# travelingspaceman/LowThrustOpt

Measured on NVIDIA B200. Metric: segment-propagations/s (fp64 state+STM), higher is better.
Workload: dtype f64

## Files before the change

lowthrustopt_b200/csrc/lto_direct_cw.cu:

```cuda
#include "lto_internal.h"
#include "lto_cw_common.cuh"
#include <algorithm>

namespace lto {

namespace cw {

constexpr int NTILE = 2;
constexpr int NSLOT = 2;
constexpr int XW0 = 2;

template <int NS>
struct Cfg {
    static constexpr int NCOL = NS + 3;
    static constexpr int NW = NTILE + NCOL;
    static constexpr int NTHREADS = 32 * NW;
    static constexpr int SVAL = (NS == 7) ? 10 : 6;
    static constexpr int OFF_H = 13 * SVAL;
    static constexpr int OFF_BM = OFF_H + 1;
    static constexpr int STEP_DOUBLES = OFF_BM + ((NS == 7) ? 3 : 0);
    static constexpr size_t REC_BYTES = (size_t)NTILE * NSLOT * STEP_DOUBLES * 32 * sizeof(double);
    static constexpr int NV = 2 * (NS + 3);
    static constexpr size_t OUT_TILE_BYTES = (size_t)16 * NS * NV * sizeof(double);
    static constexpr size_t OUT_BYTES = (size_t)NTILE * OUT_TILE_BYTES;
    static constexpr size_t BAR_OFF = REC_BYTES + OUT_BYTES;
    static constexpr size_t FLAG_OFF = BAR_OFF + (size_t)NTILE * NSLOT * 2 * sizeof(unsigned long long);
    static constexpr size_t PARK_OFF = (FLAG_OFF + (size_t)NTILE * NSLOT * sizeof(int) + 15) & ~(size_t)15;
    static constexpr int NPARK = (NS == 7) ? 7 : 6;
    static constexpr size_t SMEM = PARK_OFF + (size_t)NTILE * NCOL * NPARK * 32 * sizeof(double);
};

enum { K1P_WORK, K1P_BAR, K1P_PACE, K1P_STORE, K1P_TOTAL, K1P_STEPS, K1P_N };
#ifdef LTO_K1_PROF
constexpr int K1P_MAX_BLOCKS = 1024, K1P_MAX_WARPS = 16;
__device__ unsigned long long k1_prof[K1P_MAX_BLOCKS * K1P_MAX_WARPS * K1P_N];
struct K1Prof {
    long long c[K1P_N], t, t_begin;
    __device__ __forceinline__ void start() {
        for (int i = 0; i < K1P_N; ++i) c[i] = 0;
        t = t_begin = clock64();
    }
    __device__ __forceinline__ void mark() { t = clock64(); }
    __device__ __forceinline__ void add(int i) { const long long n = clock64(); c[i] += n - t; t = n; }
    __device__ __forceinline__ void step() { ++c[K1P_STEPS]; }
    __device__ __forceinline__ void flush(int warp, int lane) {
        c[K1P_TOTAL] = clock64() - t_begin;
        if (lane == 0 && blockIdx.x < K1P_MAX_BLOCKS)
            for (int i = 0; i < K1P_N; ++i) k1_prof[((size_t)blockIdx.x * K1P_MAX_WARPS + warp) * K1P_N + i] = (unsigned long long)c[i];
    }
};
#else
struct K1Prof {
    __device__ __forceinline__ void start() {}
    __device__ __forceinline__ void mark() {}
    __device__ __forceinline__ void add(int) {}
    __device__ __forceinline__ void step() {}
    __device__ __forceinline__ void flush(int, int) {}
};
#endif

using namespace cwc;

template <int NS, bool PUB = true>
__device__ __forceinline__ double x_step(double (&r)[3], double (&v)[3], double& m, const double (&u)[3], double omega,
                                         double mdot, double h, const EPConst& c, double* __restrict__ rec, double* __restrict__ stg,
                                         double& maxErr) {
    constexpr int SVAL = Cfg<NS>::SVAL;
    const double h2 = h * h;
    const double w2 = 2.0 * omega;
    const double kom6 = c.kthr / c.default_mass;
    double a[13][3];
    double ev[3] = {0.0, 0.0, 0.0}, ea[3] = {0.0, 0.0, 0.0};
    if (PUB) rec[Cfg<NS>::OFF_H * 32] = h;
#pragma unroll
    for (int j = 0; j < 13; ++j) {
        double R[3], V[3];
#pragma unroll
        for (int q = 0; q < 3; ++q) {
            double accv = 0.0, accr = 0.0;
#pragma unroll
            for (int l = 0; l < j; ++l) {
                if (lto_tab::Bf(j, l) != 0.0) accv = fma(lto_tab::Bf(j, l), a[l][q], accv);
                if (lto_tab::Gf(j, l) != 0.0) accr = fma(lto_tab::Gf(j, l), a[l][q], accr);
            }
            V[q] = (j == 0) ? v[q] : fma(h, accv, v[q]);
            R[q] = (j == 0) ? r[q] : fma(h2, accr, fma(h * lto_tab::Cf(j), v[q], r[q]));
        }
        const double dx1 = R[0] + c.mu, dx2 = dx1 - 1.0;
        const double yz = fma(R[1], R[1], R[2] * R[2]);
        const double i1 = fast_rsqrt(fma(dx1, dx1, yz));
        const double i2 = fast_rsqrt(fma(dx2, dx2, yz));
        const double i1s = i1 * i1, i2s = i2 * i2;
        const double a31 = c.m1 * i1s * i1, a32 = c.mu * i2s * i2;
        const double gg1 = 1.0 - (a31 + a32);
        double kom = kom6, im = 0.0;
        if (NS == 7) { im = fast_rcp(fma(h * lto_tab::Cf(j), mdot, m)); kom = c.kthr * im; }
        a[j][0] = fma(u[0], kom, fma(-a31, dx1, fma(-a32, dx2, fma(w2, V[1], R[0]))));
        a[j][1] = fma(u[1], kom, fma(gg1, R[1], -w2 * V[0]));
        a[j][2] = fma(u[2], kom, (gg1 - 1.0) * R[2]);
        if (PUB && j != 10) {
            const double a51 = 3.0 * i1s * a31, a52 = 3.0 * i2s * a32;
            const double s5 = a51 + a52;
            const double p1 = a51 * dx1, p2 = a52 * dx2;
            const double t = p1 + p2;
            const double s5y = s5 * R[1];
            double2* w = reinterpret_cast<double2*>(stg + j * SVAL * 32);
            w[0] = make_double2(fma(p1, dx1, fma(p2, dx2, gg1)), fma(s5y, R[1], gg1));
            w[1] = make_double2(fma(s5 * R[2], R[2], gg1 - 1.0), t * R[1]);
            w[2] = make_double2(t * R[2], s5y * R[2]);
            if (NS == 7) {
                const double k2 = -kom * im;
                w[3] = make_double2(kom, k2 * u[0]);
                w[4] = make_double2(k2 * u[1], k2 * u[2]);
            }
        }
        if (lto_tab::PSIf(j) != 0.0) {
#pragma unroll
            for (int q = 0; q < 3; ++q) { ev[q] = fma(lto_tab::PSIf(j), V[q], ev[q]); ea[q] = fma(lto_tab::PSIf(j), a[j][q], ea[q]); }
        }
    }
    double delta = 0.0;
#pragma unroll
    for (int q = 0; q < 3; ++q) {
        double sv = 0.0, sr = 0.0;
#pragma unroll
        for (int l = 0; l < 13; ++l) {
            if (lto_tab::CHIf(l) != 0.0) sv = fma(lto_tab::CHIf(l), a[l][q], sv);
            if (lto_tab::CHIBf(l) != 0.0) sr = fma(lto_tab::CHIBf(l), a[l][q], sr);
        }
        r[q] = fma(h2, sr, fma(h, v[q], r[q]));
        v[q] = fma(h, sv, v[q]);
        delta = fmax(delta, fmax(fabs(ev[q]), fabs(ea[q])));
    }
    if (NS == 7) m = fma(h, mdot, m);
    delta *= fabs(h * lto_tab::ERRC);
    maxErr = fmax(maxErr, delta);
    return delta;
}

template <int NS>
__device__ __forceinline__ void col_step(double (&sr)[3], double (&sv)[3], double& sm, double bm, int gc,
                                         double omega, double kom6, const double* __restrict__ rec, const double* __restrict__ stg) {
    constexpr int SVAL = Cfg<NS>::SVAL;
    constexpr bool MASS = (NS == 7);
    const double h = rec[Cfg<NS>::OFF_H * 32];
    const double h2 = h * h;
    const double w2 = 2.0 * omega;
    double a[13][3];
#pragma unroll
    for (int j = 0; j < 13; ++j) {
        if (j == 10) continue;
        double R[3], V[3];
#pragma unroll
        for (int q = 0; q < 3; ++q) {
            double accv = 0.0, accr = 0.0;
#pragma unroll
            for (int l = 0; l < j; ++l) {
                if (lto_tab::Bf(j, l) != 0.0) accv = fma(lto_tab::Bf(j, l), a[l][q], accv);
                if (lto_tab::Gf(j, l) != 0.0) accr = fma(lto_tab::Gf(j, l), a[l][q], accr);
            }
            V[q] = (j == 0) ? sv[q] : fma(h, accv, sv[q]);
            R[q] = (j == 0) ? sr[q] : fma(h2, accr, fma(h * lto_tab::Cf(j), sv[q], sr[q]));
        }
        const double2* w = reinterpret_cast<const double2*>(stg + j * SVAL * 32);
        const double2 w0 = w[0], w1 = w[1], w2v = w[2];
        const double U[6] = {w0.x, w0.y, w1.x, w1.y, w2v.x, w2v.y};
        double2 w3 = make_double2(kom6, 0.0), w4 = make_double2(0.0, 0.0);
        if (MASS) { w3 = w[3]; w4 = w[4]; }
        const double kom = w3.x;
        double acc[3];
        acc[0] = fma(w2, V[1], gc == 0 ? kom : 0.0);
        acc[1] = fma(-w2, V[0], gc == 1 ? kom : 0.0);
        acc[2] = gc == 2 ? kom : 0.0;
        if (MASS) {
            const double smj = fma(h * lto_tab::Cf(j), bm, sm);
            const double am[3] = {w3.y, w4.x, w4.y};
#pragma unroll
            for (int q = 0; q < 3; ++q) acc[q] = fma(am[q], smj, acc[q]);
        }
        sym3_mul_acc(U, R, acc);
#pragma unroll
        for (int q = 0; q < 3; ++q) a[j][q] = acc[q];
    }
#pragma unroll
    for (int q = 0; q < 3; ++q) {
        double dv = 0.0, dr = 0.0;
#pragma unroll
        for (int l = 0; l < 13; ++l) {
            if (lto_tab::CHIf(l) != 0.0) dv = fma(lto_tab::CHIf(l), a[l][q], dv);
            if (lto_tab::CHIBf(l) != 0.0) dr = fma(lto_tab::CHIBf(l), a[l][q], dr);
        }
        sr[q] = fma(h2, dr, fma(h, sv[q], sr[q]));
        sv[q] = fma(h, dv, sv[q]);
    }
    if (MASS) sm = fma(h, bm, sm);
}

struct ColState { double sr[3], sv[3], sm; };

template <int NS>
__device__ __forceinline__ void col_init(ColState& c, int col) {
#pragma unroll
    for (int q = 0; q < 3; ++q) { c.sr[q] = (col == q) ? 1.0 : 0.0; c.sv[q] = (col == q + 3) ? 1.0 : 0.0; }
    c.sm = (NS == 7 && col == 6) ? 1.0 : 0.0;
}

template <int NS>
__device__ __forceinline__ void col_park(double* __restrict__ p, const ColState& c) {
#pragma unroll
    for (int q = 0; q < 3; ++q) { p[q * 32] = c.sr[q]; p[(3 + q) * 32] = c.sv[q]; }
    if (NS == 7) p[6 * 32] = c.sm;
}

template <int NS>
__device__ __forceinline__ void col_unpark(const double* __restrict__ p, ColState& c) {
#pragma unroll
    for (int q = 0; q < 3; ++q) { c.sr[q] = p[q * 32]; c.sv[q] = p[(3 + q) * 32]; }
    c.sm = (NS == 7) ? p[6 * 32] : 0.0;
}

template <int NS>
__device__ __forceinline__ void col_store(double* __restrict__ stage, const ColState& c, int col, int lane) {
    constexpr int NV = 2 * (NS + 3);
    const int back = lane & 1, gc = col - NS;
    const int ocol = (gc >= 0) ? (2 * NS + (back ? 3 : 0) + gc) : ((back ? NS : 0) + col);
    double* J = stage + (lane >> 1) * (NS * NV) + ocol * NS;
    const double rj = (col >= 3 && col < 6) ? -1.0 : 1.0;
    const double sp = back ? -rj : 1.0;
    const double sq = back ? rj : 1.0;
    J[0] = sp * c.sr[0]; J[1] = sp * c.sr[1]; J[2] = sp * c.sr[2];
    J[3] = sq * c.sv[0]; J[4] = sq * c.sv[1]; J[5] = sq * c.sv[2];
    if (NS == 7) J[6] = sp * c.sm;
}

template <int NS>
__device__ __forceinline__ double* col_park_at(double* parks, int t, int col, int lane) {
    return parks + (size_t)(t * Cfg<NS>::NCOL + col) * Cfg<NS>::NPARK * 32 + lane;
}

template <int NS, bool ADAPT>
__device__ __forceinline__ bool col_tile_step(int t, unsigned g, int col, int gc, int lane, double omega, double kom6, double* recs, double* parks,
                                              unsigned bars, volatile int* lastf, K1Prof& pf) {
    typedef Cfg<NS> C;
    const unsigned slot = g & (NSLOT - 1), par = (g / NSLOT) & 1;
    const double* slotp = recs + (size_t)(t * NSLOT + slot) * C::STEP_DOUBLES * 32;
    const double* rec = slotp + lane;
    const unsigned full = bars + (unsigned)((t * NSLOT + slot) * 16), empty = full + 8;
    mbar_wait(full, par);
    pf.add(K1P_BAR);
    double* park = col_park_at<NS>(parks, t, col, lane);
    ColState cs;
    col_unpark<NS>(park, cs);
    const double bm = (NS == 7 && gc >= 0) ? rec[(C::OFF_BM + gc) * 32] : 0.0;
    const bool last = ADAPT && lastf[t * NSLOT + slot] != 0;
    col_step<NS>(cs.sr, cs.sv, cs.sm, bm, gc, omega, kom6, rec, slotp + lane * C::SVAL);
    mbar_arrive(empty);
    col_park<NS>(park, cs);
    pf.add(K1P_WORK);
    pf.step();
    return last;
}

template <int NS>
__device__ __forceinline__ void col_tiles_store(const DirectArgs& a, long long pair, int col, int lane, double* outs, double* parks) {
    typedef Cfg<NS> C;
    const bool leader = (col == 0 && lane == 0);
#pragma unroll 1
    for (int t = 0; t < NTILE; ++t) {
        const long long seg0 = (pair * NTILE + t) * 16;
        double* stage = outs + (size_t)t * (C::OUT_TILE_BYTES / sizeof(double));
        if (leader) bulk_store_wait_read_but<NTILE - 1>();
        asm volatile("bar.sync 2, %0;" ::"n"(32 * C::NCOL) : "memory");
        ColState cs;
        col_unpark<NS>(col_park_at<NS>(parks, t, col, lane), cs);
        col_store<NS>(stage, cs, col, lane);
        fence_proxy_async();
        asm volatile("bar.sync 2, %0;" ::"n"(32 * C::NCOL) : "memory");
        if (leader && seg0 < a.n_seg) {
            const long long nseg = (a.n_seg - seg0 < 16) ? (a.n_seg - seg0) : 16;
            bulk_store(a.jac + seg0 * (long long)(NS * C::NV), smem_u32(stage), (unsigned)(nseg * NS * C::NV * sizeof(double)));
        }
    }
}

template <int NS>
__device__ __forceinline__ void column_warp(const DirectArgs& a, long long n_tiles, int warp, int col, int lane, double* recs, double* outs, double* parks,
                                            unsigned bars) {
    typedef Cfg<NS> C;
    const int nstep = a.cfg.nsteps - 1;
    const double omega = (lane & 1) ? -1.0 : 1.0;
    const double kom6 = a.c.kthr / a.c.default_mass;
    const int gc = col - NS;
    K1Prof pf;
    pf.start();
    unsigned g = 0;
    for (long long pair = blockIdx.x; pair * NTILE < n_tiles; pair += gridDim.x) {
#pragma unroll 1
        for (int t = 0; t < NTILE; ++t) { ColState c; col_init<NS>(c, col); col_park<NS>(col_park_at<NS>(parks, t, col, lane), c); }
        for (int k = 0; k < nstep; ++k, ++g) {
            pf.mark();
#ifndef LTO_K1_NO_PACE
            asm volatile("bar.sync 3, %0;" ::"n"(32 * C::NCOL) : "memory");
#endif
            pf.add(K1P_PACE);
#pragma unroll 1
            for (int t = 0; t < NTILE; ++t) col_tile_step<NS, false>(t, g, col, gc, lane, omega, kom6, recs, parks, bars, nullptr, pf);
        }
        pf.mark();
        col_tiles_store<NS>(a, pair, col, lane, outs, parks);
        pf.add(K1P_STORE);
    }
    if (col == 0 && lane == 0) bulk_store_wait_all();
    pf.flush(warp, lane);
}

template <int NS>
__device__ __forceinline__ void state_warp(const DirectArgs& a, long long n_tiles, int warp, int t, int lane, double* recs, unsigned bars) {
    typedef Cfg<NS> C;
    const int nsteps = a.cfg.nsteps, nstep = nsteps - 1;
    const int back = lane & 1;
    const double omega = back ? -1.0 : 1.0;
    double r[3], v[3], m = a.c.default_mass, u[3], bm[3] = {0.0, 0.0, 0.0}, mdot = 0.0, t0 = 0.0, t1 = 1.0, maxErr = 0.0;
    K1Prof pf;
    pf.start();
    unsigned g = 0;
    for (long long pair = blockIdx.x; pair * NTILE < n_tiles; pair += gridDim.x) {
        const long long seg = (pair * NTILE + t) * 16 + (lane >> 1);
        {
            const long long sc = seg < a.n_seg ? seg : a.n_seg - 1;
            const long long ia = lto_node_a(sc, a.npt);
            const double* X = (back ? a.Xb : a.Xa) + ia * NS;
            const double* U = (back ? a.ub : a.ua) + ia * 3;
            r[0] = X[0]; r[1] = X[1]; r[2] = X[2];
            v[0] = X[3]; v[1] = X[4]; v[2] = X[5];
            if (back) { v[0] = -v[0]; v[1] = -v[1]; v[2] = -v[2]; }
            if (NS == 7) m = X[6];
            u[0] = U[0]; u[1] = U[1]; u[2] = U[2];
            const double ta = a.ta[ia], tb = a.tb[ia];
            t0 = ta; t1 = ta + (tb - ta) / 2.0;
            const double un = sqrt(fma(u[0], u[0], fma(u[1], u[1], u[2] * u[2])));
            mdot = -omega * un * a.c.cmdot;
            if (NS == 7) {
#pragma unroll
                for (int q = 0; q < 3; ++q) {
                    const double uh = (un > 0.0) ? u[q] / un : 1.0;
                    bm[q] = -omega * a.c.cmdot * uh;
                }
            }
            maxErr = 0.0;
        }
        for (int k = 0; k < nstep; ++k, ++g) {
            const unsigned slot = g & (NSLOT - 1), use = g / NSLOT;
            double* slotp = recs + (size_t)(t * NSLOT + slot) * C::STEP_DOUBLES * 32;
            double* rec = slotp + lane;
            const unsigned full = bars + (unsigned)((t * NSLOT + slot) * 16), empty = full + 8;
            pf.mark();
            if (use > 0) mbar_wait(empty, (use - 1) & 1);
            pf.add(K1P_BAR);
            const double h = linrange_at(t0, t1, nsteps, k + 1) - linrange_at(t0, t1, nsteps, k);
            if (NS == 7) {
#pragma unroll
                for (int q = 0; q < 3; ++q) rec[(C::OFF_BM + q) * 32] = bm[q];
            }
            x_step<NS>(r, v, m, u, omega, mdot, h, a.c, rec, slotp + lane * C::SVAL, maxErr);
            mbar_arrive(full);
            pf.add(K1P_WORK);
            pf.step();
        }
        const unsigned fullmask = 0xffffffffu;
        double xe[NS];
        xe[0] = r[0]; xe[1] = r[1]; xe[2] = r[2];
        xe[3] = back ? -v[0] : v[0]; xe[4] = back ? -v[1] : v[1]; xe[5] = back ? -v[2] : v[2];
        if (NS == 7) xe[6] = m;
        bool bad = false;
#pragma unroll
        for (int q = 0; q < NS; ++q) {
            const double other = __shfl_xor_sync(fullmask, xe[q], 1);
            const double d = xe[q] - other;
            bad |= !(d == d);
            if (!back && seg < a.n_seg) a.defect[seg * NS + q] = d;
        }
        const double me_o = __shfl_xor_sync(fullmask, maxErr, 1);
        if (!back && seg < a.n_seg) {
            if (a.errors) a.errors[seg] = fmax(maxErr, me_o);
            if (a.status) a.status[seg] = bad ? LTO_ST_NAN : LTO_OK;
        }
    }
    pf.flush(warp, lane);
}


template <int NS>
__device__ __forceinline__ void zero_step_record(double* rec, double* stg) {
    constexpr int SVAL = Cfg<NS>::SVAL;
#pragma unroll
    for (int j = 0; j < 13; ++j) {
        double2* w = reinterpret_cast<double2*>(stg + j * SVAL * 32);
#pragma unroll
        for (int p = 0; p < SVAL / 2; ++p) w[p] = make_double2(0.0, 0.0);
    }
    rec[Cfg<NS>::OFF_H * 32] = 0.0;
}

template <int NS>
__device__ __forceinline__ void state_warp_adapt(const DirectArgs& a, long long n_tiles, int t, int lane, double* recs, unsigned bars, volatile int* lastf) {
    typedef Cfg<NS> C;
    const int back = lane & 1;
    const double omega = back ? -1.0 : 1.0;
    const unsigned fullmask = 0xffffffffu;
    double r[3], v[3], m = a.c.default_mass, u[3], bm[3] = {0.0, 0.0, 0.0}, mdot = 0.0, dummy = 0.0;
    unsigned g = 0;
    for (long long pair = blockIdx.x; pair * NTILE < n_tiles; pair += gridDim.x) {
        const long long seg = (pair * NTILE + t) * 16 + (lane >> 1);
        const long long sc = seg < a.n_seg ? seg : a.n_seg - 1;
        const long long ia = lto_node_a(sc, a.npt);
        const double* X = (back ? a.Xb : a.Xa) + ia * NS;
        const double* U = (back ? a.ub : a.ua) + ia * 3;
        r[0] = X[0]; r[1] = X[1]; r[2] = X[2];
        v[0] = X[3]; v[1] = X[4]; v[2] = X[5];
        if (back) { v[0] = -v[0]; v[1] = -v[1]; v[2] = -v[2]; }
        if (NS == 7) m = X[6];
        u[0] = U[0]; u[1] = U[1]; u[2] = U[2];
        const double ta = a.ta[ia], tb = a.tb[ia];
        const double t0 = ta, tfinal = ta + (tb - ta) / 2.0;
        const double un = sqrt(fma(u[0], u[0], fma(u[1], u[1], u[2] * u[2])));
        mdot = -omega * un * a.c.cmdot;
        if (NS == 7) {
#pragma unroll
            for (int q = 0; q < 3; ++q) { const double uh = (un > 0.0) ? u[q] / un : 1.0; bm[q] = -omega * a.c.cmdot * uh; }
        }
        const double hmax = (tfinal - t0) / 2.5, hmin = (tfinal - t0) / 1e7;
        double tt = t0, h = (tfinal - t0) / 50.0;
        int status = 0, nt = 0;
        bool done = !((tt < tfinal) && (h >= hmin));
        while (true) {
            const unsigned slot = g & (NSLOT - 1), use = g / NSLOT;
            double* slotp = recs + (size_t)(t * NSLOT + slot) * C::STEP_DOUBLES * 32;
            double* rec = slotp + lane;
            double* stg = slotp + lane * C::SVAL;
            const unsigned full = bars + (unsigned)((t * NSLOT + slot) * 16), empty = full + 8;
            if (use > 0) mbar_wait(empty, (use - 1) & 1);
            if (NS == 7) {
#pragma unroll
                for (int q = 0; q < 3; ++q) rec[(C::OFF_BM + q) * 32] = bm[q];
            }
            bool pending = !done;
            if (done) {
                zero_step_record<NS>(rec, stg);
            }
            while (__any_sync(fullmask, pending)) {
                if (pending) {
                    if (tt + h > tfinal) h = tfinal - tt;
                    if (nt >= a.cfg.max_attempts) { status = LTO_ST_MAXSTEPS; done = true; pending = false; }
                }
                if (pending) {
                    ++nt;
                    double r2[3] = {r[0], r[1], r[2]}, v2[3] = {v[0], v[1], v[2]}, m2 = m;
                    const double xn = fmax(fmax(fmax(fabs(r[0]), fabs(r[1])), fmax(fabs(r[2]), fabs(v[0]))), fmax(fmax(fabs(v[1]), fabs(v[2])), NS == 7 ? fabs(m) : 0.0));
                    double delta = x_step<NS>(r2, v2, m2, u, omega, mdot, h, a.c, rec, stg, dummy);
                    if (!(delta == delta)) { status = LTO_ST_NAN; done = true; pending = false; }
                    else {
                        const double tau = a.cfg.tol * fmax(xn, 1.0);
                        if (delta <= tau) {
                            tt += h;
                            r[0] = r2[0]; r[1] = r2[1]; r[2] = r2[2]; v[0] = v2[0]; v[1] = v2[1]; v[2] = v2[2]; m = m2;
                            pending = false;
                        }
                        if (delta == 0.0) delta = 1e-16;
                        h = fmin(hmax, 0.8 * h * pow(tau / delta, 0.125));
                        if (!((tt < tfinal) && (h >= hmin))) { done = true; if (pending) { status = LTO_ST_HMIN; pending = false; } }
                    }
                }
            }
            if (status != 0) zero_step_record<NS>(rec, stg);
            const bool all_done = __all_sync(fullmask, done);
            if (lane == 0) lastf[t * NSLOT + slot] = all_done ? 1 : 0;
            mbar_arrive(full);
            ++g;
            if (all_done) break;
        }
        if (status == 0 && tt < tfinal) status = LTO_ST_HMIN;
        double xe[NS];
        xe[0] = r[0]; xe[1] = r[1]; xe[2] = r[2];
        xe[3] = back ? -v[0] : v[0]; xe[4] = back ? -v[1] : v[1]; xe[5] = back ? -v[2] : v[2];
        if (NS == 7) xe[6] = m;
        bool bad = false;
#pragma unroll
        for (int q = 0; q < NS; ++q) {
            const double other = __shfl_xor_sync(fullmask, xe[q], 1);
            const double d = xe[q] - other;
            bad |= !(d == d);
            if (!back && seg < a.n_seg) a.defect[seg * NS + q] = d;
        }
        const int st_o = __shfl_xor_sync(fullmask, status, 1);
        if (!back && seg < a.n_seg) {
            if (a.errors) a.errors[seg] = 0.0;
            if (a.status) a.status[seg] = status ? status : (st_o ? st_o : (bad ? LTO_ST_NAN : LTO_OK));
        }
    }
}

template <int NS>
__device__ __forceinline__ void column_warp_adapt(const DirectArgs& a, long long n_tiles, int warp, int col, int lane, double* recs, double* outs,
                                                  double* parks, unsigned bars, volatile int* lastf) {
    const double omega = (lane & 1) ? -1.0 : 1.0;
    const double kom6 = a.c.kthr / a.c.default_mass;
    const int gc = col - NS;
    K1Prof pf;
    pf.start();
    unsigned g[NTILE];
#pragma unroll
    for (int t = 0; t < NTILE; ++t) g[t] = 0;
    for (long long pair = blockIdx.x; pair * NTILE < n_tiles; pair += gridDim.x) {
#pragma unroll 1
        for (int t = 0; t < NTILE; ++t) { ColState c; col_init<NS>(c, col); col_park<NS>(col_park_at<NS>(parks, t, col, lane), c); }
        unsigned alive = (1u << NTILE) - 1u;
        while (alive) {
            pf.mark();
#ifndef LTO_K1_NO_PACE
            asm volatile("bar.sync 3, %0;" ::"n"(32 * Cfg<NS>::NCOL) : "memory");
#endif
            pf.add(K1P_PACE);
#pragma unroll
            for (int t = 0; t < NTILE; ++t) {
                if (!(alive & (1u << t))) continue;
                if (col_tile_step<NS, true>(t, g[t], col, gc, lane, omega, kom6, recs, parks, bars, lastf, pf)) alive &= ~(1u << t);
                ++g[t];
            }
        }
        pf.mark();
        col_tiles_store<NS>(a, pair, col, lane, outs, parks);
        pf.add(K1P_STORE);
    }
    if (col == 0 && lane == 0) bulk_store_wait_all();
    pf.flush(warp, lane);
}

template <int NS, bool ADAPT>
__global__ void __launch_bounds__(Cfg<NS>::NTHREADS, 1) k_direct_cw(DirectArgs a, long long n_tiles) {
    typedef Cfg<NS> C;
    extern __shared__ __align__(16) unsigned char smem_raw[];
    double* recs = reinterpret_cast<double*>(smem_raw);
    double* outs = reinterpret_cast<double*>(smem_raw + C::REC_BYTES);
    double* parks = reinterpret_cast<double*>(smem_raw + C::PARK_OFF);
    const unsigned bars = smem_u32(smem_raw + C::BAR_OFF);
    const int warp = threadIdx.x >> 5, lane = threadIdx.x & 31;
    if (threadIdx.x == 0) {
#pragma unroll
        for (int i = 0; i < NTILE * NSLOT; ++i) {
            mbar_init(bars + i * 16, 32);
            mbar_init(bars + i * 16 + 8, 32 * C::NCOL);
        }
    }
    __syncthreads();
    volatile int* lastf = reinterpret_cast<volatile int*>(smem_raw + C::FLAG_OFF);
    if (warp >= XW0 && warp < XW0 + NTILE) {
        if (ADAPT) state_warp_adapt<NS>(a, n_tiles, warp - XW0, lane, recs, bars, lastf);
        else state_warp<NS>(a, n_tiles, warp, warp - XW0, lane, recs, bars);
    } else {
        const int col = warp < XW0 ? warp : warp - NTILE;
        if (ADAPT) column_warp_adapt<NS>(a, n_tiles, warp, col, lane, recs, outs, parks, bars, lastf);
        else column_warp<NS>(a, n_tiles, warp, col, lane, recs, outs, parks, bars);
    }
}

template <int NS>
__global__ void __launch_bounds__(128) k_direct_state(DirectArgs a) {
    const int nsteps = a.cfg.nsteps, nstep = nsteps - 1;
    const int lane = threadIdx.x & 31, back = lane & 1;
    const double omega = back ? -1.0 : 1.0;
    const long long n_pairs32 = (a.n_seg + 15) / 16;
    const long long warp0 = ((long long)blockIdx.x * blockDim.x + threadIdx.x) >> 5, nwarp = ((long long)gridDim.x * blockDim.x) >> 5;
    for (long long w = warp0; w < n_pairs32; w += nwarp) {
        const long long seg = w * 16 + (lane >> 1);
        const long long sc = seg < a.n_seg ? seg : a.n_seg - 1;
        const long long ia = lto_node_a(sc, a.npt);
        const double* X = (back ? a.Xb : a.Xa) + ia * NS;
        const double* U = (back ? a.ub : a.ua) + ia * 3;
        double r[3] = {X[0], X[1], X[2]}, v[3] = {X[3], X[4], X[5]}, m = a.c.default_mass, u[3] = {U[0], U[1], U[2]}, maxErr = 0.0;
        if (back) { v[0] = -v[0]; v[1] = -v[1]; v[2] = -v[2]; }
        if (NS == 7) m = X[6];
        const double ta = a.ta[ia], tb = a.tb[ia];
        const double t0 = ta, t1 = ta + (tb - ta) / 2.0;
        const double un = sqrt(fma(u[0], u[0], fma(u[1], u[1], u[2] * u[2])));
        const double mdot = -omega * un * a.c.cmdot;
        for (int k = 0; k < nstep; ++k) {
            const double h = linrange_at(t0, t1, nsteps, k + 1) - linrange_at(t0, t1, nsteps, k);
            x_step<NS, false>(r, v, m, u, omega, mdot, h, a.c, nullptr, nullptr, maxErr);
        }
        const unsigned fullmask = 0xffffffffu;
        double xe[NS];
        xe[0] = r[0]; xe[1] = r[1]; xe[2] = r[2];
        xe[3] = back ? -v[0] : v[0]; xe[4] = back ? -v[1] : v[1]; xe[5] = back ? -v[2] : v[2];
        if (NS == 7) xe[6] = m;
        bool bad = false;
#pragma unroll
        for (int q = 0; q < NS; ++q) {
            const double other = __shfl_xor_sync(fullmask, xe[q], 1);
            const double d = xe[q] - other;
            bad |= !(d == d);
            if (!back && seg < a.n_seg) a.defect[seg * NS + q] = d;
        }
        const double me_o = __shfl_xor_sync(fullmask, maxErr, 1);
        if (!back && seg < a.n_seg) {
            if (a.errors) a.errors[seg] = fmax(maxErr, me_o);
            if (a.status) a.status[seg] = bad ? LTO_ST_NAN : LTO_OK;
        }
    }
}

}

template <int NS>
static cudaError_t launch_state(const DirectArgs& a, cudaStream_t st) {
    int dev = 0, n_sm = 0;
    cudaError_t e = cudaGetDevice(&dev); if (e != cudaSuccess) return e;
    e = cudaDeviceGetAttribute(&n_sm, cudaDevAttrMultiProcessorCount, dev); if (e != cudaSuccess) return e;
    const long long n_warps = (a.n_seg + 15) / 16;
    const long long blocks = (n_warps + 3) / 4;
    const int grid = (int)std::min<long long>(blocks, (long long)n_sm * 16);
    cw::k_direct_state<NS><<<grid, 128, 0, st>>>(a);
    return cudaGetLastError();
}

template <int NS, bool ADAPT>
static cudaError_t launch_cw(const DirectArgs& a, cudaStream_t st) {
    typedef cw::Cfg<NS> C;
    static int n_sm_dev[64] = {0};
    static bool attr_dev[64] = {false};
    int dev = 0;
    { cudaError_t e = cudaGetDevice(&dev); if (e != cudaSuccess) return e; }
    if (dev < 0 || dev >= 64) return cudaErrorInvalidDevice;
    if (!attr_dev[dev]) {
        cudaError_t e = cudaDeviceGetAttribute(&n_sm_dev[dev], cudaDevAttrMultiProcessorCount, dev); if (e != cudaSuccess) return e;
        e = cudaFuncSetAttribute(cw::k_direct_cw<NS, ADAPT>, cudaFuncAttributeMaxDynamicSharedMemorySize, (int)C::SMEM);
        if (e != cudaSuccess) return e;
        attr_dev[dev] = true;
    }
    const int n_sm = n_sm_dev[dev];
    const long long n_tiles = (a.n_seg + 15) / 16;
    const long long n_pairs = (n_tiles + cw::NTILE - 1) / cw::NTILE;
    const int grid = (int)std::min<long long>(n_pairs, (long long)n_sm);
    cw::k_direct_cw<NS, ADAPT><<<grid, C::NTHREADS, C::SMEM, st>>>(a, n_tiles);
    return cudaGetLastError();
}

#ifdef LTO_K1_PROF
extern "C" int lto_k1_prof_read(unsigned long long* out, int n_words) {
    const size_t n = std::min<size_t>((size_t)n_words, sizeof(cw::k1_prof) / sizeof(unsigned long long));
    return (int)cudaMemcpyFromSymbol(out, cw::k1_prof, n * sizeof(unsigned long long));
}
#endif

cudaError_t launch_direct_cw(const DirectArgs& a, int nstate, cudaStream_t st, int* n_launch) {
    *n_launch = 0;
    if (a.n_seg <= 0 || a.n_seg > (1ll << 34)) return cudaErrorNotSupported;
    if (a.cfg.mode != 0 && (a.cfg.err_norm != 0 || a.jac == nullptr)) return cudaErrorNotSupported;
    if (a.jac != nullptr && (reinterpret_cast<uintptr_t>(a.jac) & 15u) != 0) return cudaErrorNotSupported;
    cudaError_t e;
    if (a.jac == nullptr) {
        if (nstate == 7) e = launch_state<7>(a, st);
        else if (nstate == 6) e = launch_state<6>(a, st);
        else return cudaErrorNotSupported;
    } else if (a.cfg.mode != 0) {
        if (nstate == 7) e = launch_cw<7, true>(a, st);
        else if (nstate == 6) e = launch_cw<6, true>(a, st);
        else return cudaErrorNotSupported;
    } else if (nstate == 7) e = launch_cw<7, false>(a, st);
    else if (nstate == 6) e = launch_cw<6, false>(a, st);
    else return cudaErrorNotSupported;
    if (e == cudaSuccess) *n_launch = 1;
    return e;
}

}
```

Measured before the change: 100.8 million.

## Prefetch next segment inputs with cp.async and shuffle-based step sizes

State warps now stage the next tile's node state, control, and time bounds into a new shared-memory 'legs' buffer with cp.async while the current tile propagates. This hides global-load latency at tile boundaries. Step sizes are computed once per 32 steps as lane-parallel linrange values and broadcast with shuffles instead of two linrange_at calls per step. The bm writes are also limited to the first NSLOT steps, and column warps switch to a parked mbarrier wait. Costs are extra shared memory and a reliance on recycled slots still holding the earlier bm values.

```diff
diff --git a/lowthrustopt_b200/csrc/lto_direct_cw.cu b/lowthrustopt_b200/csrc/lto_direct_cw.cu
--- a/lowthrustopt_b200/csrc/lto_direct_cw.cu
+++ b/lowthrustopt_b200/csrc/lto_direct_cw.cu
@@ -27,7 +27,10 @@
     static constexpr size_t FLAG_OFF = BAR_OFF + (size_t)NTILE * NSLOT * 2 * sizeof(unsigned long long);
     static constexpr size_t PARK_OFF = (FLAG_OFF + (size_t)NTILE * NSLOT * sizeof(int) + 15) & ~(size_t)15;
     static constexpr int NPARK = (NS == 7) ? 7 : 6;
-    static constexpr size_t SMEM = PARK_OFF + (size_t)NTILE * NCOL * NPARK * 32 * sizeof(double);
+    static constexpr size_t LEGS_OFF = PARK_OFF + (size_t)NTILE * NCOL * NPARK * 32 * sizeof(double);
+    static constexpr int NLEG = NS + 5;
+    static constexpr size_t SMEM = LEGS_OFF + (size_t)NLEG * NTILE * 32 * sizeof(double);
+    static_assert(SMEM <= 227 * 1024, "K1 / K2 shared memory exceeds a block's limit");
 };
 
 enum { K1P_WORK, K1P_BAR, K1P_PACE, K1P_STORE, K1P_TOTAL, K1P_STEPS, K1P_N };
@@ -60,6 +63,64 @@
 #endif
 
 using namespace cwc;
+
+__device__ __forceinline__ void cp_async8(double* dst, const double* src) {
+    asm volatile("cp.async.ca.shared.global [%0], [%1], 8;" ::"r"(smem_u32(dst)), "l"(src) : "memory");
+}
+
+__device__ __forceinline__ unsigned legs_slot() {
+    unsigned tid;
+    asm volatile("mov.u32 %0, %%tid.x;" : "=r"(tid));
+    return tid - 32 * XW0;
+}
+
+template <int NS>
+__device__ __forceinline__ void legs_prefetch(const DirectArgs& a, long long seg, double* legs) {
+    const long long sc = seg < a.n_seg ? seg : a.n_seg - 1;
+    const long long ia = lto_node_a(sc, a.npt);
+    const unsigned i = legs_slot();
+    const int back = i & 1;
+    const double* X = (back ? a.Xb : a.Xa) + ia * NS;
+    const double* U = (back ? a.ub : a.ua) + ia * 3;
+    double* d = legs + i;
+    constexpr int LS = NTILE * 32;
+#pragma unroll
+    for (int k = 0; k < NS; ++k) cp_async8(d + k * LS, X + k);
+#pragma unroll
+    for (int q = 0; q < 3; ++q) cp_async8(d + (NS + q) * LS, U + q);
+    cp_async8(d + (NS + 3) * LS, a.ta + ia);
+    cp_async8(d + (NS + 4) * LS, a.tb + ia);
+    asm volatile("cp.async.commit_group;" ::: "memory");
+}
+
+template <int NS>
+__device__ __forceinline__ void legs_take(const double* legs, const EPConst& c, double (&r)[3], double (&v)[3], double& m, double (&u)[3],
+                                          double (&bm)[3], double& mdot, double& t0, double& t1) {
+    asm volatile("cp.async.wait_all;" ::: "memory");
+    const unsigned i = legs_slot();
+    const double* s = legs + i;
+    constexpr int LS = NTILE * 32;
+    const int back = i & 1;
+    const double omega = back ? -1.0 : 1.0;
+    r[0] = s[0]; r[1] = s[LS]; r[2] = s[2 * LS];
+    v[0] = s[3 * LS]; v[1] = s[4 * LS]; v[2] = s[5 * LS];
+    if (back) { v[0] = -v[0]; v[1] = -v[1]; v[2] = -v[2]; }
+    if (NS == 7) m = s[6 * LS];
+    u[0] = s[NS * LS]; u[1] = s[(NS + 1) * LS]; u[2] = s[(NS + 2) * LS];
+    const double ta = s[(NS + 3) * LS], tb = s[(NS + 4) * LS];
+    t0 = ta; t1 = ta + (tb - ta) / 2.0;
+    const double un = sqrt(fma(u[0], u[0], fma(u[1], u[1], u[2] * u[2])));
+    mdot = -omega * un * c.cmdot;
+    if (NS == 7) {
+#pragma unroll
+        for (int q = 0; q < 3; ++q) {
+            const double uh = (un > 0.0) ? u[q] / un : 1.0;
+            bm[q] = -omega * c.cmdot * uh;
+        }
+    }
+}
+
+__device__ __forceinline__ double linrange_lerp(double a, double b, double t) { return (1.0 - t) * a + t * b; }
 
 template <int NS, bool PUB = true>
 __device__ __forceinline__ double x_step(double (&r)[3], double (&v)[3], double& m, const double (&u)[3], double omega,
@@ -246,7 +307,7 @@
     const double* slotp = recs + (size_t)(t * NSLOT + slot) * C::STEP_DOUBLES * 32;
     const double* rec = slotp + lane;
     const unsigned full = bars + (unsigned)((t * NSLOT + slot) * 16), empty = full + 8;
-    mbar_wait(full, par);
+    mbar_wait_parked(full, par);
     pf.add(K1P_BAR);
     double* park = col_park_at<NS>(parks, t, col, lane);
     ColState cs;
@@ -315,40 +376,26 @@
 }
 
 template <int NS>
-__device__ __forceinline__ void state_warp(const DirectArgs& a, long long n_tiles, int warp, int t, int lane, double* recs, unsigned bars) {
+__device__ __forceinline__ void state_warp(const DirectArgs& a, long long n_tiles, int warp, int t, int lane, double* recs, double* legs,
+                                           unsigned bars) {
     typedef Cfg<NS> C;
     const int nsteps = a.cfg.nsteps, nstep = nsteps - 1;
     const int back = lane & 1;
     const double omega = back ? -1.0 : 1.0;
+    const unsigned fullmask = 0xffffffffu;
+    const double tw0 = (double)lane / (double)(nsteps - 1);
     double r[3], v[3], m = a.c.default_mass, u[3], bm[3] = {0.0, 0.0, 0.0}, mdot = 0.0, t0 = 0.0, t1 = 1.0, maxErr = 0.0;
     K1Prof pf;
     pf.start();
     unsigned g = 0;
+    if ((long long)blockIdx.x * NTILE < n_tiles) legs_prefetch<NS>(a, ((long long)blockIdx.x * NTILE + t) * 16 + (lane >> 1), legs);
     for (long long pair = blockIdx.x; pair * NTILE < n_tiles; pair += gridDim.x) {
         const long long seg = (pair * NTILE + t) * 16 + (lane >> 1);
-        {
-            const long long sc = seg < a.n_seg ? seg : a.n_seg - 1;
-            const long long ia = lto_node_a(sc, a.npt);
-            const double* X = (back ? a.Xb : a.Xa) + ia * NS;
-            const double* U = (back ? a.ub : a.ua) + ia * 3;
-            r[0] = X[0]; r[1] = X[1]; r[2] = X[2];
-            v[0] = X[3]; v[1] = X[4]; v[2] = X[5];
-            if (back) { v[0] = -v[0]; v[1] = -v[1]; v[2] = -v[2]; }
-            if (NS == 7) m = X[6];
-            u[0] = U[0]; u[1] = U[1]; u[2] = U[2];
-            const double ta = a.ta[ia], tb = a.tb[ia];
-            t0 = ta; t1 = ta + (tb - ta) / 2.0;
-            const double un = sqrt(fma(u[0], u[0], fma(u[1], u[1], u[2] * u[2])));
-            mdot = -omega * un * a.c.cmdot;
-            if (NS == 7) {
-#pragma unroll
-                for (int q = 0; q < 3; ++q) {
-                    const double uh = (un > 0.0) ? u[q] / un : 1.0;
-                    bm[q] = -omega * a.c.cmdot * uh;
-                }
-            }
-            maxErr = 0.0;
-        }
+        legs_take<NS>(legs, a.c, r, v, m, u, bm, mdot, t0, t1);
+        if ((pair + gridDim.x) * NTILE < n_tiles) legs_prefetch<NS>(a, seg + (long long)gridDim.x * (NTILE * 16), legs);
+        maxErr = 0.0;
+        double tw = tw0;
+        double xk = linrange_lerp(t0, t1, __shfl_sync(fullmask, tw, 0));
         for (int k = 0; k < nstep; ++k, ++g) {
             const unsigned slot = g & (NSLOT - 1), use = g / NSLOT;
             double* slotp = recs + (size_t)(t * NSLOT + slot) * C::STEP_DOUBLES * 32;
@@ -357,8 +404,12 @@
             pf.mark();
             if (use > 0) mbar_wait(empty, (use - 1) & 1);
             pf.add(K1P_BAR);
-            const double h = linrange_at(t0, t1, nsteps, k + 1) - linrange_at(t0, t1, nsteps, k);
-            if (NS == 7) {
+            const int j = k + 1;
+            if ((j & 31) == 0) tw = (double)(j + lane) / (double)(nsteps - 1);
+            const double xj = linrange_lerp(t0, t1, __shfl_sync(fullmask, tw, j & 31));
+            const double h = xj - xk;
+            xk = xj;
+            if (NS == 7 && k < NSLOT) {
 #pragma unroll
                 for (int q = 0; q < 3; ++q) rec[(C::OFF_BM + q) * 32] = bm[q];
             }
@@ -367,7 +418,6 @@
             pf.add(K1P_WORK);
             pf.step();
         }
-        const unsigned fullmask = 0xffffffffu;
         double xe[NS];
         xe[0] = r[0]; xe[1] = r[1]; xe[2] = r[2];
         xe[3] = back ? -v[0] : v[0]; xe[4] = back ? -v[1] : v[1]; xe[5] = back ? -v[2] : v[2];
@@ -403,32 +453,19 @@
 }
 
 template <int NS>
-__device__ __forceinline__ void state_warp_adapt(const DirectArgs& a, long long n_tiles, int t, int lane, double* recs, unsigned bars, volatile int* lastf) {
+__device__ __forceinline__ void state_warp_adapt(const DirectArgs& a, long long n_tiles, int t, int lane, double* recs, double* legs, unsigned bars,
+                                                 volatile int* lastf) {
     typedef Cfg<NS> C;
     const int back = lane & 1;
     const double omega = back ? -1.0 : 1.0;
     const unsigned fullmask = 0xffffffffu;
-    double r[3], v[3], m = a.c.default_mass, u[3], bm[3] = {0.0, 0.0, 0.0}, mdot = 0.0, dummy = 0.0;
+    double r[3], v[3], m = a.c.default_mass, u[3], bm[3] = {0.0, 0.0, 0.0}, mdot = 0.0, t0 = 0.0, tfinal = 1.0, dummy = 0.0;
     unsigned g = 0;
+    if ((long long)blockIdx.x * NTILE < n_tiles) legs_prefetch<NS>(a, ((long long)blockIdx.x * NTILE + t) * 16 + (lane >> 1), legs);
     for (long long pair = blockIdx.x; pair * NTILE < n_tiles; pair += gridDim.x) {
         const long long seg = (pair * NTILE + t) * 16 + (lane >> 1);
-        const long long sc = seg < a.n_seg ? seg : a.n_seg - 1;
-        const long long ia = lto_node_a(sc, a.npt);
-        const double* X = (back ? a.Xb : a.Xa) + ia * NS;
-        const double* U = (back ? a.ub : a.ua) + ia * 3;
-        r[0] = X[0]; r[1] = X[1]; r[2] = X[2];
-        v[0] = X[3]; v[1] = X[4]; v[2] = X[5];
-        if (back) { v[0] = -v[0]; v[1] = -v[1]; v[2] = -v[2]; }
-        if (NS == 7) m = X[6];
-        u[0] = U[0]; u[1] = U[1]; u[2] = U[2];
-        const double ta = a.ta[ia], tb = a.tb[ia];
-        const double t0 = ta, tfinal = ta + (tb - ta) / 2.0;
-        const double un = sqrt(fma(u[0], u[0], fma(u[1], u[1], u[2] * u[2])));
-        mdot = -omega * un * a.c.cmdot;
-        if (NS == 7) {
-#pragma unroll
-            for (int q = 0; q < 3; ++q) { const double uh = (un > 0.0) ? u[q] / un : 1.0; bm[q] = -omega * a.c.cmdot * uh; }
-        }
+        legs_take<NS>(legs, a.c, r, v, m, u, bm, mdot, t0, tfinal);
+        if ((pair + gridDim.x) * NTILE < n_tiles) legs_prefetch<NS>(a, seg + (long long)gridDim.x * (NTILE * 16), legs);
         const double hmax = (tfinal - t0) / 2.5, hmin = (tfinal - t0) / 1e7;
         double tt = t0, h = (tfinal - t0) / 50.0;
         int status = 0, nt = 0;
@@ -555,8 +592,9 @@
     __syncthreads();
     volatile int* lastf = reinterpret_cast<volatile int*>(smem_raw + C::FLAG_OFF);
     if (warp >= XW0 && warp < XW0 + NTILE) {
-        if (ADAPT) state_warp_adapt<NS>(a, n_tiles, warp - XW0, lane, recs, bars, lastf);
-        else state_warp<NS>(a, n_tiles, warp, warp - XW0, lane, recs, bars);
+        double* legs = reinterpret_cast<double*>(smem_raw + C::LEGS_OFF);
+        if (ADAPT) state_warp_adapt<NS>(a, n_tiles, warp - XW0, lane, recs, legs, bars, lastf);
+        else state_warp<NS>(a, n_tiles, warp, warp - XW0, lane, recs, legs, bars);
     } else {
         const int col = warp < XW0 ? warp : warp - NTILE;
         if (ADAPT) column_warp_adapt<NS>(a, n_tiles, warp, col, lane, recs, outs, parks, bars, lastf);
```

New measurement: 100.6 million, median of 6. No clear change (-0.2%).
